# kostastril/Aiyagari-Replication

Hardware: AMD Instinct MI355X
Metric: Bellman evals/sec (Na·Na'·Nz, fp64) (higher is better)
Workload: dtype f64; 1 GPU; aiyagari_vfi_sweep Na=20000 Nz=7 rouwenhorst (BASELINE configs[1]); Na=20000, Nz=7, search=exhaustive over a' (exact bound-tree screen)

## Files before the change

### aiyagari-replication_amd/csrc/bell_dev.hpp

```cpp
#pragma once
#include <hip/hip_runtime.h>

#include "aiy_common.hpp"

namespace aiy {

constexpr double kTau = 1.4210854715202004e-14;
constexpr double kThr = 0.99999999999999644729;
constexpr float kThr32 = 0.999998092651367f;
constexpr float kBig32 = 1.152921504606847e18f;

typedef float f32x2 __attribute__((ext_vector_type(2)));

__device__ __forceinline__ float f32_up(double x) { return nextafterf((float)x, __builtin_inff()); }
__device__ __forceinline__ float f32_dn(double x) { return nextafterf((float)x, -__builtin_inff()); }

template <int NP>
__device__ __forceinline__ f32x2 ipow2(f32x2 c) {
    static_assert(NP >= 1 && NP <= 8, "screen exponent");
    if constexpr (NP == 1) return c;
    f32x2 c2 = c * c;
    if constexpr (NP == 2) return c2;
    if constexpr (NP == 3) return c2 * c;
    f32x2 c4 = c2 * c2;
    if constexpr (NP == 4) return c4;
    if constexpr (NP == 5) return c4 * c;
    if constexpr (NP == 6) return c4 * c2;
    if constexpr (NP == 7) return (c4 * c2) * c;
    return c4 * c4;
}

template <int NP, bool LAB>
__device__ __forceinline__ double bell_val(double c, double ev, double sigma, double dis) {
    double u;
    if constexpr (NP > 0) {
        double p = 1.0 / aiy_ipow(c, NP);
        if constexpr ((NP & (NP - 1)) == 0)
            u = (p - 1) * (-1.0 / NP);
        else
            u = (p - 1) / (1 - sigma);
    } else {
        if (!LAB && sigma == 1.0) u = aiy_log(c);
        else u = (aiy_pow(c, 1.0 - sigma) - 1) / (1 - sigma);
    }
    if constexpr (LAB) return (u - dis) + ev;
    else return u + ev;
}

#define AIY_SCHED_BARRIER() __builtin_amdgcn_sched_barrier(0)
template <int NP, int M, bool CLAMP = true>
__device__ __forceinline__ void screen_t(double (&t)[M], const double (&cx)[M],
                                         const double (&dd)[M]) {
    double c[M], p[M];
#pragma unroll
    for (int m = 0; m < M; ++m) c[m] = CLAMP ? fmax(cx[m], 0.0) : cx[m];
    if constexpr (CLAMP) AIY_SCHED_BARRIER();
#pragma unroll
    for (int m = 0; m < M; ++m) p[m] = c[m];
    constexpr int top = 31 - __builtin_clz((unsigned)NP);
#pragma unroll
    for (int b = top - 1; b >= 0; --b) {
#pragma unroll
        for (int m = 0; m < M; ++m) p[m] = p[m] * p[m];
        AIY_SCHED_BARRIER();
        if ((NP >> b) & 1) {
#pragma unroll
            for (int m = 0; m < M; ++m) p[m] = p[m] * c[m];
            AIY_SCHED_BARRIER();
        }
    }
#pragma unroll
    for (int m = 0; m < M; ++m) t[m] = dd[m] * p[m];
}
__device__ __forceinline__ double clamp0_d(double x) {
#if defined(__HIP_DEVICE_COMPILE__)
    double r;
    asm("v_max_f64 %0, %1, 0" : "=v"(r) : "v"(x));
    return r;
#else
    return fmax(x, 0.0);
#endif
}
template <int RL>
struct StageGroup {
    static constexpr int G = RL <= 2 ? 8 : (RL <= 4 ? 4 : 1);
};

__device__ __forceinline__ bool lexi_take(double val, int q, double& best, int& idx) {
    if (val != val) return false;
    if (idx < 0 || val > best || (val == best && q < idx)) {
        best = val;
        idx = q;
        return true;
    }
    return false;
}

__device__ __forceinline__ void lexi_take_sel(double val, int q, double& best, int& idx) {
    const bool take = (val == val) & ((idx < 0) | (val > best) | ((val == best) & (q < idx)));
    best = take ? val : best;
    idx = take ? q : idx;
}

__device__ __forceinline__ double screen_B(double best, int idx, double dis, int np) {
    if (idx < 0) return -__builtin_inf();
    double nd = (double)np;
    return nd * (best + dis) - kTau * nd * (fabs(best) + fabs(dis));
}

__device__ __forceinline__ double wave_fmin_d(double x) {
    x = fmin(x, dpp_d<0xB1>(x));
    x = fmin(x, dpp_d<0x4E>(x));
    x = fmin(x, dpp_d<0x141>(x));
    x = fmin(x, dpp_d<0x140>(x));
    x = fmin(x, dpp_d<0x142, 0xa>(x));
    x = fmin(x, dpp_d<0x143, 0xc>(x));
    return readlane_d(x, 63);
}
__device__ __forceinline__ double wave_fmax_d(double x) {
    x = fmax(x, dpp_d<0xB1>(x));
    x = fmax(x, dpp_d<0x4E>(x));
    x = fmax(x, dpp_d<0x141>(x));
    x = fmax(x, dpp_d<0x140>(x));
    x = fmax(x, dpp_d<0x142, 0xa>(x));
    x = fmax(x, dpp_d<0x143, 0xc>(x));
    return readlane_d(x, 63);
}

constexpr int kTreeGroup = 8;

__device__ __forceinline__ double group_fmin_d(double x) {
    x = fmin(x, dpp_d<0xB1>(x));
    x = fmin(x, dpp_d<0x4E>(x));
    return fmin(x, dpp_d<0x141>(x));
}
__device__ __forceinline__ double group_fmax_d(double x) {
    x = fmax(x, dpp_d<0xB1>(x));
    x = fmax(x, dpp_d<0x4E>(x));
    return fmax(x, dpp_d<0x141>(x));
}
__device__ __forceinline__ double wave_rest_fmin_d(double x) {
    x = fmin(x, dpp_d<0x140>(x));
    x = fmin(x, dpp_d<0x142, 0xa>(x));
    x = fmin(x, dpp_d<0x143, 0xc>(x));
    return readlane_d(x, 63);
}
__device__ __forceinline__ double wave_rest_fmax_d(double x) {
    x = fmax(x, dpp_d<0x140>(x));
    x = fmax(x, dpp_d<0x142, 0xa>(x));
    x = fmax(x, dpp_d<0x143, 0xc>(x));
    return readlane_d(x, 63);
}

template <int NP>
__device__ __forceinline__ bool screen_wave(double dmax, double a0, double bmin, double cmax) {
    const double cx[1] = {cmax - a0}, dd[1] = {dmax - bmin};
    double t[1];
    screen_t<NP, 1>(t, cx, dd);
    return t[0] >= kThr;
}

template <bool LAB>
__device__ __forceinline__ double cash(double x, double y, double Ll) {
    if constexpr (LAB) return x + y * Ll;
    else return x + y;
}

__device__ __forceinline__ double table_ev(int N, int Na, const double* __restrict__ P,
                                           const double* __restrict__ V, double beta, int i,
                                           int k) {
    double acc = 0.0;
    for (int m0 = 0; m0 < N; m0 += 8) {
        double pm[8], vv[8];
#pragma unroll
        for (int u = 0; u < 8; ++u) {
            const int m = min(m0 + u, N - 1);
            pm[u] = P[i * N + m];
            vv[u] = V[(size_t)m * Na + k];
        }
#pragma unroll
        for (int u = 0; u < 8; ++u) {
            const double term = (beta * pm[u]) * vv[u];
            acc = acc + (m0 + u < N ? term : 0.0);
        }
    }
    return acc;
}
__device__ __forceinline__ double table_D(double ev, int np) {
    double ne = (double)np * ev;
    return (ne + 1.0) + kTau * (fabs(ne) + 1.0);
}

}
```

### aiyagari-replication_amd/csrc/bellman_kernels.hip

```cpp
#include <hip/hip_ext.h>

#include <algorithm>
#include <type_traits>

#include "aiy_common.hpp"
#include "bell_dev.hpp"
#include "bellman.hpp"

namespace aiy {

__device__ __forceinline__ BellArgs bell_cand(const BellArgs& A, int c) {
    BellArgs B = A;
    const size_t o = (size_t)c * A.N * A.Na;
    B.r = A.rv[c];
    B.w = A.wv[c];
    B.v_old += o;
    B.EV += o;
    if (B.Dt) B.Dt += o;
    if (B.Dm8) B.Dm8 += (size_t)c * A.N * A.nb8;
    if (B.Dm512) B.Dm512 += (size_t)c * A.N * A.nb512;
    B.kf += o * A.Nl;
    B.best0 += o;
    B.idx0 += o;
    if (B.hint) B.hint += o;
// ... 537 lines not shown
        const int gb = (k_lo >> 6) + g + lane;
        const bool okb = g + lane < nbk;
        const double dmv = okb ? Dmrow[gb] : -__builtin_inf();
        const double a0v = okb ? a[gb << 6] : 0.0;
        double smv = dmv;
        smv = fmax(smv, __shfl_xor(smv, 1));
        smv = fmax(smv, __shfl_xor(smv, 2));
        smv = fmax(smv, __shfl_xor(smv, 4));
        const int ng = min(64, nbk - g);
        for (int sb = 0; sb < ng; sb += 8) {
            ++nsup;
            if (!bound_pass(readlane_d(smv, sb), readlane_d(a0v, sb))) continue;
            const int se = min(sb + 8, ng);
            for (int b = sb; b < se; ++b) {
                if (se - sb > 1) {
                    ++nblk;
                    if (!bound_pass(readlane_d(dmv, b), readlane_d(a0v, b))) continue;
                }
                const int b0 = k_lo + ((g + b) << 6);
                fine(b0, min(b0 + 64, k_hi));
            }
        }
    }
    if (A.hitcount) {
        const unsigned ns = 64 * R * (l1 - l0);
        nsup *= ns;
        nblk *= ns;
    }

    const size_t slab = ((size_t)lbk * nchunk + chunk) * N + i;
#pragma unroll
    for (int r = 0; r < R; ++r) {
        int j = jbase + r * 64 + lane;
        if (j < Na && imp[r] >= 0) {
            A.partial[slab * Na + j] = imp[r];
            A.touched[(size_t)i * Na + j] = 1;
        }
    }
    if (A.hitcount) {
        unsigned long long* hc = A.hitcount + 4 * (item % kDiffSlots);
        if (nhits) atomicAdd(hc, (unsigned long long)nhits);
        if (lane == 0) {
            atomicAdd(hc + 1, (unsigned long long)nsup);
            atomicAdd(hc + 2, (unsigned long long)nblk);
            if (nfine) atomicAdd(hc + 3, (unsigned long long)nfine * 64 * R * (l1 - l0));
        }
    }
}

template <int NP, bool LAB, int R, int LB, int W, bool INS, int PK, bool HY = false, int WM = 8>
__device__ __forceinline__ void bell_tree_item(const BellArgs& A0, int ntile, int block_id,
                                               int nblocks, double2 (*s_cand)[512],
                                               unsigned long long* s_pass) {
    static_assert(PK == 1 || W == 1, "packed workgroups hold one-wave tiles");
    const int lane = threadIdx.x & 63;
    const int lw = readfirst(threadIdx.x >> 6);
    const int wave = PK > 1 ? 0 : lw;
    asm volatile("" ::"s"(A0.a), "s"(A0.Dt), "s"(A0.EV), "s"(A0.kf), "s"(A0.hint), "s"(A0.v_old),
                 "s"(A0.Dm512), "s"(A0.s), "s"(A0.r), "s"(A0.w), "s"(A0.N), "s"(A0.Na),
                 "s"(A0.variant), "s"(A0.C), "s"(A0.nb512), "s"(A0.sigma), "s"(A0.trace),
                 "s"(A0.best0), "s"(A0.idx0), "s"(A0.tw), "s"(ntile), "s"(nblocks), "s"(A0.mom),
                 "s"(A0.idx), "s"(A0.pk), "s"(A0.pc), "s"(A0.v_new), "s"(A0.diff));
    const long long t_boot = (INS && A0.trace) ? (long long)wall_clock64() : 0;
    const long long c_boot = (INS && A0.trace) ? (long long)__builtin_amdgcn_s_memtime() : 0;
    int item = A0.perm ? A0.perm[block_id]
                       : ((A0.variant & kVarXcdOrder) ? xcd_remap(block_id, nblocks) : block_id);
    if (PK > 1 && item < 0) return;
    BellArgs A = A0;
    if (A0.C > 1) {
        const int c = item / (A0.N * ntile);
        if (A0.stop[c]) return;
        A = bell_cand(A0, c);
        item -= c * A0.N * ntile;
    }
    const int tile = item % ntile;
    const int i = item / ntile;
    const int N = A.N, Na = A.Na, Nl = LAB ? A.Nl : 1;
    const size_t nall = (size_t)N * Na;
    const double* __restrict__ a = A.a;
    const double* __restrict__ Drow = A.Dt + (size_t)i * Na;
    const double* __restrict__ ev = A.EV + (size_t)i * Na;
    const double y = A.w * A.s[i];
    const int TW = (R == 1 && A0.tw > 0) ? A0.tw : 64 * R;
    const int jbase = tile * TW;
    constexpr bool LEAN = (W >= 2 && !HY) || LAB;

    int* __restrict__ mom = (A.variant & kVarNoMomentum) ? nullptr : A.mom;
    constexpr bool PRE = WM == 1;
    int h_pre[R], m_pre[R], kf_pre[R];
    double aj_pre[R];
    if constexpr (PRE) {
#pragma unroll
        for (int r = 0; r < R; ++r) {
            const int j = jbase + r * 64 + lane;
            const int jc = (j < Na && r * 64 + lane < TW) ? j : 0;
            const size_t t = (size_t)i * Na + jc;
            h_pre[r] = A.hint ? A.hint[t] : -1;
            m_pre[r] = (A.hint && mom) ? mom[t] : 0;
            kf_pre[r] = A.kf[t];
            aj_pre[r] = a[jc];
        }
    }
    double dm0_pre, a0_pre;
    {
        const bool oks = lane < A.nb512;
        dm0_pre = oks ? A.Dm512[(size_t)i * A.nb512 + lane] : -__builtin_inf();
        a0_pre = oks ? a[lane << 9] : 0.0;
    }
    double vo_pre[R];
#pragma unroll
    for (int r = 0; r < R; ++r) {
        const int j = jbase + r * 64 + lane;
        vo_pre[r] = (j < Na && r * 64 + lane < TW && wave == 0) ? A.v_old[(size_t)i * Na + j] : 0.0;
    }

    double x[R], best[R];
    int idx[R], hk0[R], mlast[R];
    bool okr[R], feas[R];
    unsigned nsu = 0;
#pragma unroll
    for (int r = 0; r < R; ++r) {
        const int j = jbase + r * 64 + lane;
        okr[r] = j < Na && r * 64 + lane < TW;
        const size_t t = (size_t)i * Na + (okr[r] ? j : 0);
        if constexpr (PRE) x[r] = okr[r] ? (1 + A.r) * aj_pre[r] : 0.0;
        else x[r] = okr[r] ? (1 + A.r) * a[j] : 0.0;
        best[r] = __builtin_nan("");
        idx[r] = -1;
        hk0[r] = -1;
        mlast[r] = 0;
        feas[r] = false;
        if (!okr[r]) continue;
        if constexpr (PRE) feas[r] = kf_pre[r] > 0;
        for (int l = PRE ? 1 : 0; l < Nl; ++l) feas[r] = feas[r] || A.kf[l * nall + t] > 0;
        if (A.hint) {
            int h;
            if constexpr (PRE) h = h_pre[r];
            else h = A.hint[t];
            int mraw = 0;
            if constexpr (PRE) mraw = h >= 0 ? m_pre[r] : 0;
            else mraw = (mom && h >= 0) ? mom[t] : 0;
            const int ms0 = (int)(short)(mraw & 0xffff), ms1 = (int)(short)(mraw >> 16);
            mlast[r] = ms0;
            const int mv = max(-Na, min(Na, (A.variant & kVarDriftExtrap) ? 2 * ms0 - ms1 : ms0));
            if (h >= 0) {
                const int hl = h % Nl;
                const int kf = (PRE && hl == 0) ? kf_pre[r] : A.kf[hl * nall + t];
                if (kf > 0) {
                    const int hk = min(h / Nl, kf - 1);
                    const double coh = cash<LAB>(x[r], y, LAB ? A.L[hl] : 1.0);
                    const double dis = LAB ? A.dis[hl] : 0.0;
                    auto take = [&](int k) __attribute__((always_inline)) {
                        if (INS) ++nsu;
                        return lexi_take(bell_val<NP, LAB>(coh - a[k], ev[k], A.sigma, dis),
                                         hl + Nl * k, best[r], idx[r]);
                    };
                    const int wn =
                        WM == 1 ? 1 : 1 << ((A.variant & kVarHintWinMask) >> kVarHintWinShift);
                    hk0[r] = hk;
                    const int hm = min(max(hk + mv, 0), kf - 1);
                    constexpr int mw = 1;
                    const bool usem = hm > hk + wn + mw || hm < hk - wn - mw;
                    const int wnh = (usem && (A.variant & kVarHintAlone)) ? 0 : wn;
                    const bool skiph = usem && (A.variant & kVarNoHintEval);
                    double wa[2 * WM + 1], we[2 * WM + 1], ma[3], me[3];
#pragma unroll
                    for (int d = -WM; d <= WM; ++d) {
                        if (d < -wnh || d > wnh || skiph) continue;
                        const int kc = min(max(hk + d, 0), kf - 1);
                        wa[d + WM] = a[kc];
                        we[d + WM] = ev[kc];
                    }
                    if (usem) {
#pragma unroll
                        for (int d = -1; d <= 1; ++d) {
                            const int kc = min(max(hm + d, 0), kf - 1);
                            ma[d + 1] = a[kc];
                            me[d + 1] = ev[kc];
                        }
                    }
#pragma unroll
                    for (int d = -WM; d <= WM; ++d) {
                        if (d < -wnh || d > wnh || skiph) continue;
                        const int kc = min(max(hk + d, 0), kf - 1);
                        if (INS) ++nsu;
                        lexi_take(bell_val<NP, LAB>(coh - wa[d + WM], we[d + WM], A.sigma, dis),
                                  hl + Nl * kc, best[r], idx[r]);
                    }
                    if (usem) {
#pragma unroll
                        for (int d = -1; d <= 1; ++d) {
                            const int kc = min(max(hm + d, 0), kf - 1);
                            if (INS) ++nsu;
                            lexi_take(bell_val<NP, LAB>(coh - ma[d + 1], me[d + 1], A.sigma, dis),
                                      hl + Nl * kc, best[r], idx[r]);
                        }
                    }
                    const int kb = idx[r] >= 0 ? idx[r] / Nl : hk;
                    int dir = kb >= hk + wnh ? 1 : (kb <= hk - wnh ? -1 : 0);
                    if (usem && kb >= hm - mw && kb <= hm + mw)
                        dir = kb == hm + mw ? 1 : (kb == hm - mw ? -1 : 0);
                    if (dir != 0 && !(A.variant & kVarNoClimb)) {
                        int k = kb, step = 2;
                        for (;;) {
                            const int kn = min(max(k + dir * step, 0), kf - 1);
                            if (kn == k || !take(kn)) break;
                            k = kn;
                            step <<= 1;
                        }
                        for (int s2 = step >> 1; s2 >= 1; s2 >>= 1) {
                            const int c0 = idx[r] / Nl;
                            if (c0 + s2 < kf) take(c0 + s2);
                            if (c0 - s2 >= 0) take(c0 - s2);
                        }
                    }
                }
            }
        } else {
            best[r] = A.best0[t];
            idx[r] = A.idx0[t] == -2 ? -1 : A.idx0[t];
        }
    }
    int q_su[R];
    double kp_su[R];
#pragma unroll
    for (int r = 0; r < R; ++r) {
        q_su[r] = idx[r];
        kp_su[r] = a[idx[r] >= 0 ? idx[r] / Nl : 0];
    }
    unsigned nhits = nsu, nsup = 0, nwv = 0, nblk = 0, ngt = 0, nfine = 0, lane_pairs = 0;
    unsigned npath[2] = {0, 0};
    const long long t_start = (INS && A.trace) ? (long long)wall_clock64() : 0;
    long long cyc[4] = {0, 0, 0, 0}, c_mark = (INS && A.trace) ? (long long)__builtin_amdgcn_s_memtime() : 0;
    const long long c_mark0 = c_mark;
    auto stamp = [&](int ph) __attribute__((always_inline)) {
        if (INS && A.trace) {
            const long long now = (long long)__builtin_amdgcn_s_memtime();
            cyc[ph] += now - c_mark;
            c_mark = now;
        }
    };
    stamp(0);

    auto exchange = [&]() __attribute__((always_inline)) {
        if constexpr (W > 1) {
#pragma unroll
            for (int r = 0; r < R; ++r)
                s_cand[lw][r * 64 + lane] = make_double2(best[r], (double)idx[r]);
            __syncthreads();
            for (int v = 0; v < W; ++v)
#pragma unroll
                for (int r = 0; r < R; ++r) {
                    const double2 e = s_cand[v][r * 64 + lane];
                    if (v != wave && (int)e.y >= 0) lexi_take(e.x, (int)e.y, best[r], idx[r]);
                }
            __syncthreads();
        }
    };

    for (int l0 = 0; l0 < Nl; l0 += LB) {
        double coh[R][LB], B[R][LB], dis[LB];
        int kg = 0;
        int kfl = 0x7fffffff;
#pragma unroll
        for (int q = 0; q < LB; ++q) dis[q] = (LAB && l0 + q < Nl) ? A.dis[l0 + q] : 0.0;
#pragma unroll
        for (int r = 0; r < R; ++r) {
            const size_t t = (size_t)i * Na + (okr[r] ? jbase + r * 64 + lane : 0);
#pragma unroll
            for (int q = 0; q < LB; ++q) {
                const bool okq = okr[r] && l0 + q < Nl;
                coh[r][q] = okq ? cash<LAB>(x[r], y, LAB ? A.L[l0 + q] : 1.0) : 0.0;
                if (okq) {
                    const int kfv = A.kf[(l0 + q) * nall + t];
                    kg = max(kg, kfv);
                    kfl = min(kfl, kfv);
                }
            }
        }
        constexpr bool FAST = !LAB && R == 1;
        int kfmin = 0;
        if constexpr (FAST)
            if (!(A.variant & kVarPlainScreens)) kfmin = min(wave_min_i32(kfl), Na);
        if (A.r > -1.0) {
            const int jl = min(Na - 1, jbase + TW - 1);
            kg = readlane_i(kg, (jl - jbase) & 63);
        } else {
            for (int off = 32; off > 0; off >>= 1) kg = max(kg, __shfl_xor(kg, off));
            kg = readfirst(kg);
        }
        if (kg == 0) continue;
        if (l0 > 0) exchange();
        auto set_B = [&]() __attribute__((always_inline)) {
#pragma unroll
            for (int r = 0; r < R; ++r)
#pragma unroll
                for (int q = 0; q < LB; ++q)
                    B[r][q] = (okr[r] && l0 + q < Nl) ? screen_B(best[r], idx[r], dis[q], NP)
                                                      : __builtin_nan("");
        };
        set_B();
        constexpr bool GRP = !LAB;
        constexpr int GL = kTreeGroup;
        double gB = __builtin_nan(""), gC = -__builtin_inf();
        auto set_G = [&]() __attribute__((always_inline)) {
            double bl = __builtin_nan(""), cl = -__builtin_inf();
#pragma unroll
            for (int r = 0; r < R; ++r)
#pragma unroll
                for (int q = 0; q < LB; ++q) {
                    bl = fmin(bl, B[r][q]);
                    cl = fmax(cl, (okr[r] && l0 + q < Nl) ? coh[r][q] : -__builtin_inf());
                }
            gB = group_fmin_d(bl);
            gC = group_fmax_d(cl);
        };
        if constexpr (GRP) set_G();

        constexpr int RL = R * LB, G = LEAN ? (RL <= 2 ? 4 : 1) : StageGroup<RL>::G;
        auto mask8 = [&](double dv, double av, int l0, int stride, int cnt, bool sub = false)
                         __attribute__((always_inline)) {
            double dmax[8], a0[8];
#pragma unroll
            for (int u = 0; u < 8; ++u) {
                const int ln = min(l0 + stride * u, 63);
                dmax[u] = readlane_d(dv, ln);
                a0[u] = readlane_d(av, ln);
            }
            bool pu[8];
#pragma unroll
            for (int g0 = 0; g0 < 8; g0 += G) {
                double cx[G * RL], dd[G * RL], t[G * RL];
#pragma unroll
                for (int gu = 0; gu < G; ++gu)
#pragma unroll
                    for (int r = 0; r < R; ++r)
#pragma unroll
                        for (int q = 0; q < LB; ++q) {
                            const int m = (gu * R + r) * LB + q;
                            cx[m] = coh[r][q] - a0[g0 + gu];
                            dd[m] = dmax[g0 + gu] - B[r][q];
                        }
                AIY_SCHED_BARRIER();
                screen_t<NP, G * RL>(t, cx, dd);
#pragma unroll
                for (int gu = 0; gu < G; ++gu) {
                    bool pass = false;
#pragma unroll
                    for (int m = gu * RL; m < (gu + 1) * RL; ++m) pass = pass || t[m] >= kThr;
                    pu[g0 + gu] = pass;
                }
            }
            unsigned m = 0;
#pragma unroll
            for (int u = 0; u < 8; ++u) m |= (__any(pu[u]) ? 1u : 0u) << u;
            if (INS && A.trace && sub)
#pragma unroll
                for (int u = 0; u < 8; ++u) lane_pairs += (u < cnt && pu[u]) ? 1u : 0u;
            return m & ((1u << cnt) - 1u);
        };
        auto load_tk = [&](int bit, double2 (&tk)[8]) __attribute__((always_inline)) {
#pragma unroll
            for (int kk = 0; kk < 8; ++kk) tk[kk] = s_cand[lw][(bit << 3) + kk];
        };
        auto fine = [&](int sbase, int k0, int k1, const double2 (&tk)[8])
                        __attribute__((always_inline)) {
            if (INS && (A.hitcount || A.trace)) nfine += k1 - k0;
            const bool ncl = FAST && k0 + 8 <= kfmin;
            if (INS && A.hitcount) npath[0] += ncl ? 0u : 1u, npath[1] += ncl ? 1u : 0u;
            bool pk[8];
#pragma unroll
            for (int g0 = 0; g0 < 8; g0 += G) {
                double cx[G * RL], dd[G * RL], t[G * RL];
#pragma unroll
                for (int gk = 0; gk < G; ++gk)
#pragma unroll
                    for (int r = 0; r < R; ++r)
#pragma unroll
                        for (int q = 0; q < LB; ++q) {
                            const int m = (gk * R + r) * LB + q;
                            cx[m] = coh[r][q] - tk[g0 + gk].x;
                            dd[m] = tk[g0 + gk].y - B[r][q];
                        }
                AIY_SCHED_BARRIER();
                if constexpr (FAST) {
                    if (!ncl) {
#pragma unroll
                        for (int m = 0; m < G * RL; ++m) cx[m] = clamp0_d(cx[m]);
                        AIY_SCHED_BARRIER();
                    }
                    screen_t<NP, G * RL, false>(t, cx, dd);
                } else {
                    screen_t<NP, G * RL>(t, cx, dd);
                }
#pragma unroll
                for (int gk = 0; gk < G; ++gk) {
                    bool pass = false;
#pragma unroll
                    for (int r = 0; r < R; ++r)
#pragma unroll
                        for (int q = 0; q < LB; ++q) {
                            const int lin = (l0 + q) + Nl * (k0 + g0 + gk);
                            pass = pass || (t[(gk * R + r) * LB + q] >= kThr && lin != idx[r]);
                        }
                    pk[g0 + gk] = pass;
                }
            }
            {
                bool pall = false;
#pragma unroll
                for (int kk = 0; kk < 8; ++kk) pall = pall || pk[kk];
                if (!__any(pall)) return;
            }
            unsigned vote = 0;
#pragma unroll
            for (int kk = 0; kk < 8; ++kk) vote |= (__any(pk[kk]) ? 1u : 0u) << kk;
            vote &= (1u << (k1 - k0)) - 1u;
            if (!vote) return;
            stamp(2);
            while (vote) {
                const int kk = __builtin_ctz(vote);
                vote &= vote - 1;
                const int k = k0 + kk;
                const double2 tkk = s_cand[lw][k - sbase];
#pragma unroll
                for (int r = 0; r < R; ++r)
#pragma unroll
                    for (int q = 0; q < LB; ++q) {
                        const double c = coh[r][q] - tkk.x;
                        const int lin = (l0 + q) + Nl * k;
                        if (lin != idx[r] && c > 0 &&
                            (tkk.y - B[r][q]) * aiy_ipow(c, NP) >= kThr) {
                            ++nhits;
                            const double val =
                                bell_val<NP, LAB>(c, ev[k], A.sigma, dis[q]);
                            if (lexi_take(val, lin, best[r], idx[r])) {
#pragma unroll
                                for (int q2 = 0; q2 < LB; ++q2)
                                    if (B[r][q2] == B[r][q2])
                                        B[r][q2] = screen_B(best[r], idx[r], dis[q2], NP);
                            }
                        }
                    }
            }
            stamp(3);
        };
        auto load8 = [&](int sb, double& dm8, double& a8) __attribute__((always_inline)) {
            const int sub = (sb << 6) + lane;
            const bool oku = sub < A.nb8;
            dm8 = oku ? A.Dm8[(size_t)i * A.nb8 + sub] : -__builtin_inf();
            a8 = oku ? a[sub << 3] : 0.0;
        };
        auto stage = [&](int sbase, unsigned long long pass, double2 (&st)[8])
                         __attribute__((always_inline)) {
            if constexpr (LEAN) {
                unsigned bm = 0;
#pragma unroll
                for (int b = 0; b < 8; ++b) bm |= ((pass >> (8 * b)) & 0xffull) ? 1u << b : 0u;
                while (bm) {
                    const int b0 = __builtin_ctz(bm);
                    bm &= bm - 1;
                    const int b1 = bm ? __builtin_ctz(bm) : -1;
                    if (bm) bm &= bm - 1;
                    const int k0 = min(sbase + (b0 << 6) + lane, Na - 1);
                    const double2 v0 = make_double2(a[k0], Drow[k0]);
                    double2 v1 = make_double2(0.0, 0.0);
                    if (b1 >= 0) {
                        const int k1 = min(sbase + (b1 << 6) + lane, Na - 1);
                        v1 = make_double2(a[k1], Drow[k1]);
                    }
                    s_cand[lw][(b0 << 6) + lane] = v0;
                    if (b1 >= 0) s_cand[lw][(b1 << 6) + lane] = v1;
                }
            } else {
#pragma unroll
                for (int b = 0; b < 8; ++b)
                    if ((pass >> (8 * b)) & 0xffull) {
                        const int k = min(sbase + (b << 6) + lane, Na - 1);
                        st[b] = make_double2(a[k], Drow[k]);
                    }
            }
        };
        auto prep = [&](int sb, int bsel, int bstep, double dm8, double a8, double2 (&st)[8],
                        bool subsplit = false)
                        __attribute__((always_inline)) -> unsigned long long {
            stamp(0);
            const int sbase = sb << 9;
            if constexpr (GRP) {
                constexpr int NG = 64 / GL, CH = LEAN ? 4 : 8;
                static_assert(NG % CH == 0, "whole chunks of groups");
                unsigned long long any = 0;
#pragma unroll
                for (int g0 = 0; g0 < NG; g0 += CH) {
                    double cx[CH], dd[CH], t[CH];
#pragma unroll
                    for (int u = 0; u < CH; ++u) {
                        cx[u] = readlane_d(gC, (g0 + u) * GL) - a8;
                        dd[u] = dm8 - readlane_d(gB, (g0 + u) * GL);
                    }
                    AIY_SCHED_BARRIER();
                    screen_t<NP, CH>(t, cx, dd);
#pragma unroll
                    for (int u = 0; u < CH; ++u) any |= __ballot(t[u] >= kThr);
                }
                if (INS && (A.hitcount || A.trace)) ngt += NG;
                const int nfe = min(64, (kg - sbase + 7) >> 3);
                unsigned long long pass = any & (nfe >= 64 ? ~0ull : (1ull << nfe) - 1ull);
                if (bstep > 1) {
                    const unsigned long long one = subsplit ? 0x01ull : 0xffull;
                    unsigned long long pat = one << (subsplit ? bsel : 8 * bsel);
                    for (int sh = subsplit ? bstep : 8 * bstep; sh < 64; sh <<= 1) pat |= pat << sh;
                    pass &= pat;
                }
                if (INS && (A.hitcount || A.trace)) nblk += __builtin_popcountll(pass);
                unsigned long long keep = 0;
                for (unsigned long long m = pass; m; m &= m - 1) {
                    const int u = __builtin_ctzll(m);
                    const double dv = readlane_d(dm8, u), av = readlane_d(a8, u);
                    double cx[RL], dd[RL], t[RL];
#pragma unroll
                    for (int r = 0; r < R; ++r)
#pragma unroll
                        for (int q = 0; q < LB; ++q) {
                            cx[r * LB + q] = coh[r][q] - av;
                            dd[r * LB + q] = dv - B[r][q];
                        }
                    screen_t<NP, RL>(t, cx, dd);
                    bool p = false;
#pragma unroll
                    for (int m2 = 0; m2 < RL; ++m2) p = p || t[m2] >= kThr;
                    if (__any(p)) keep |= 1ull << u;
                }
                pass = keep;
                if (INS && A.trace && lane == 0) lane_pairs += __builtin_popcountll(pass);
                stage(sbase, pass, st);
                stamp(1);
                return pass;
            }
            double dm64 = dm8;
            dm64 = fmax(dm64, dpp_d<0xB1>(dm64));
            dm64 = fmax(dm64, dpp_d<0x4E>(dm64));
            dm64 = fmax(dm64, dpp_d<0x104>(dm64));
            const int nblock = min(8, (kg - sbase + 63) >> 6);
            unsigned own = 0;
            for (int b = subsplit ? 0 : bsel; b < nblock; b += subsplit ? 1 : bstep) own |= 1u << b;
            if (INS && (A.hitcount || A.trace)) nblk += __builtin_popcount(own);
            const unsigned bpass = mask8(dm64, a8, 0, 8, nblock) & own;
            unsigned long long pass = 0;
            const bool deal = subsplit && bstep > 1;
            int ord = 0;
            for (unsigned bm = bpass; bm; bm &= bm - 1, ++ord) {
                if (deal && ord % bstep != bsel) continue;
                const int b = __builtin_ctz(bm);
                const int nsub = min(8, (kg - (sbase + (b << 6)) + 7) >> 3);
                if (INS && (A.hitcount || A.trace)) nblk += nsub;
                pass |= (unsigned long long)mask8(dm8, a8, 8 * b, 1, nsub, true) << (8 * b);
            }
            if constexpr (W > 1) {
                if (deal) {
                    s_pass[bsel] = pass;
                    __syncthreads();
                    unsigned long long all = 0;
                    for (int v = 0; v < bstep; ++v) all |= s_pass[v];
                    __syncthreads();
                    const unsigned long long pat = bstep == 2 ? 0x5555555555555555ull
                                                 : (bstep == 4 ? 0x1111111111111111ull
                                                               : 0x0101010101010101ull);
                    pass = all & (pat << bsel);
                }
            }
            stage(sbase, pass, st);
            stamp(1);
            return pass;
        };
        auto finish = [&](int sb, unsigned long long pass, const double2 (&st)[8])
                          __attribute__((always_inline)) {
            const int sbase = sb << 9;
            if constexpr (!LEAN)
#pragma unroll
                for (int b = 0; b < 8; ++b)
                    if ((pass >> (8 * b)) & 0xffull) s_cand[lw][(b << 6) + lane] = st[b];
            __builtin_amdgcn_wave_barrier();
            __builtin_amdgcn_fence(__ATOMIC_RELEASE, "wavefront");
            stamp(1);
            double2 tkA[8], tkB[8];
            unsigned long long pm = pass;
            if constexpr (LEAN) {
                for (; pm; pm &= pm - 1) {
                    const int b0 = __builtin_ctzll(pm);
                    load_tk(b0, tkA);
                    fine(sbase, sbase + (b0 << 3), min(sbase + (b0 << 3) + 8, kg), tkA);
                }
            }
            if (pm) load_tk(__builtin_ctzll(pm), tkA);
            while (pm) {
                const int b0 = __builtin_ctzll(pm);
                pm &= pm - 1;
                if (pm) load_tk(__builtin_ctzll(pm), tkB);
                fine(sbase, sbase + (b0 << 3), min(sbase + (b0 << 3) + 8, kg), tkA);
                if (!pm) break;
                const int b1 = __builtin_ctzll(pm);
                pm &= pm - 1;
                if (pm) load_tk(__builtin_ctzll(pm), tkA);
                fine(sbase, sbase + (b1 << 3), min(sbase + (b1 << 3) + 8, kg), tkB);
            }
            stamp(2);
            __builtin_amdgcn_wave_barrier();
        };

        const int nsb = (kg + 511) >> 9;
        int sfirst = -1;
        {
            int hk = -1;
#pragma unroll
            for (int r = 0; r < R; ++r)
                if (idx[r] >= 0) hk = idx[r] / Nl;
            const unsigned long long m = __ballot(hk >= 0);
            if (m) sfirst = min(readlane_i(hk, __builtin_ctzll(m)) >> 9, nsb - 1);
        }
        double2 st_cur[8], st_prev[8];
        if (sfirst >= 0) {
            if (INS) ++nsup;
            double d8, a8;
            load8(sfirst, d8, a8);
            const unsigned long long p = prep(sfirst, wave, W, d8, a8, st_cur,
                                              (A.variant & kVarDealBlocks) != 0);
            if (p) finish(sfirst, p, st_cur);
            exchange();
            set_B();
        }
        double dm0, a0;
        auto load512 = [&](int g) __attribute__((always_inline)) {
            const int sbl = g + lane;
            const bool oks = sbl < nsb;
            dm0 = oks ? A.Dm512[(size_t)i * A.nb512 + sbl] : -__builtin_inf();
            a0 = oks ? a[sbl << 9] : 0.0;
        };
        if (l0 == 0) {
            dm0 = dm0_pre;
            a0 = a0_pre;
        } else {
            load512(0);
        }
        double bmin, cmax;
        {
            if constexpr (GRP) {
                if (sfirst >= 0) set_G();
                bmin = wave_rest_fmin_d(gB);
                cmax = wave_rest_fmax_d(gC);
            } else {
                double bl = __builtin_nan(""), cl = -__builtin_inf();
#pragma unroll
                for (int r = 0; r < R; ++r)
#pragma unroll
                    for (int q = 0; q < LB; ++q) {
                        bl = fmin(bl, B[r][q]);
                        cl = fmax(cl, (okr[r] && l0 + q < Nl) ? coh[r][q] : -__builtin_inf());
                    }
                bmin = wave_fmin_d(bl);
                cmax = wave_fmax_d(cl);
            }
        }
        int g = 0;
        unsigned long long sm = 0;
        auto test512 = [&]() __attribute__((always_inline)) {
            if (INS) ++nwv;
            unsigned long long m =
                __ballot(lane < nsb - g && screen_wave<NP>(dm0, a0, bmin, cmax));
            static_assert(64 % W == 0, "superblock g + u belongs to wave u % W");
            if constexpr (W > 1) m &= (~0ull / ((1ull << W) - 1ull)) << wave;
            if (sfirst >= g && sfirst < g + 64) m &= ~(1ull << (sfirst - g));
            return m;
        };
        if (nsb > 0) sm = test512();
        auto next_sb = [&]() __attribute__((always_inline)) -> int {
            for (;;) {
                if (sm) {
                    const int u = __builtin_ctzll(sm);
                    sm &= sm - 1;
                    if (INS) ++nsup;
                    return g + u;
                }
                g += 64;
                if (g >= nsb) return -1;
                load512(g);
                sm = test512();
            }
        };
        int cur = nsb > 0 ? next_sb() : -1;
        double pd = 0.0, pa = 0.0;
        if (cur >= 0) load8(cur, pd, pa);
        unsigned long long pass_prev = 0;
        int sb_prev = -1;
        while (cur >= 0) {
            const double d8 = pd, a8 = pa;
            const int nxt = next_sb();
            if (nxt >= 0) load8(nxt, pd, pa);
            const unsigned long long pc = prep(cur, 0, 1, d8, a8, st_cur);
            if constexpr (LEAN) {
                if (pc) finish(cur, pc, st_cur);
                cur = nxt;
                continue;
            }
            if (pass_prev) finish(sb_prev, pass_prev, st_prev);
#pragma unroll
            for (int b = 0; b < 8; ++b) st_prev[b] = st_cur[b];
            pass_prev = pc;
            sb_prev = cur;
            cur = nxt;
        }
        if (pass_prev) finish(sb_prev, pass_prev, st_prev);
    }

    exchange();
    const long long c_end = (INS && A.trace) ? (long long)__builtin_amdgcn_s_memtime() : 0;

    bool okd = false;
    double dmax = 0.0;
#pragma unroll
    for (int r = 0; r < R; ++r) {
        if (!okr[r] || wave != 0) continue;
        const size_t t = (size_t)i * Na + jbase + r * 64 + lane;
        double b = best[r];
        int q = idx[r];
        const double vo = vo_pre[r];
        if (!feas[r] && LAB) {
            b = A.keep_incoming ? A.v_new[t] : vo;
        } else {
            if (q < 0) {
                q = 0;
                b = __builtin_nan("");
            }
            const int l = q % Nl, k = q / Nl;
            double kp = kp_su[r];
            if (__ballot(q != q_su[r]) != 0ull) kp = a[k];
            A.idx[t] = q;
            if (A.pk) A.pk[t] = kp;
            if (A.pc) A.pc[t] = cash<LAB>(x[r], y, LAB ? A.L[l] : 1.0) - kp;
            if (LAB && A.pl) A.pl[t] = A.L[l];
        }
        A.v_new[t] = b;
        if (mom && A.hint) {
            const int sh = (hk0[r] >= 0 && idx[r] >= 0) ? idx[r] / Nl - hk0[r] : 0;
            const int shc = max(-32767, min(32767, sh));
            mom[t] = (int)(((unsigned)shc & 0xffffu) | ((unsigned)mlast[r] << 16));
        }
        const double d = fabs(b - vo);
        if (d == d) {
            dmax = okd ? fmax(dmax, d) : d;
            okd = true;
        }
    }
    if constexpr (W == 1) wave_max_to_slots(okd, dmax, A.diff);
    else block_max_to_slots(okd, dmax, A.diff);
    if (INS && A.trace) {
        __shared__ unsigned s_cnt[W][4];
        __shared__ unsigned s_pairs;
        static_assert(LAB || 8 % (R * LB) == 0, "group tests in whole block-test units");
        const unsigned nblk_all = nblk + ngt / (R * LB);
        unsigned pairs = lane_pairs, sums[4] = {nsup, nblk_all, nfine, nhits};
        if constexpr (W == 1) {
            for (int o = 32; o > 0; o >>= 1) pairs += __shfl_xor(pairs, o);
        } else {
            if (threadIdx.x == 0) s_pairs = 0;
            __syncthreads();
            atomicAdd(&s_pairs, lane_pairs);
            if (lane == 0) {
                s_cnt[wave][0] = nsup; s_cnt[wave][1] = nblk_all; s_cnt[wave][2] = nfine; s_cnt[wave][3] = nhits;
            }
            __syncthreads();
            pairs = s_pairs;
            for (int c = 0; c < 4; ++c) {
                unsigned sum = 0;
                for (int v = 0; v < W; ++v) sum += s_cnt[v][c];
                sums[c] = sum;
            }
        }
        if (W == 1 ? lane == 0 : threadIdx.x == 0) {
            long long* tr = A.trace + 16 * (size_t)item;
            tr[0] = t_start;
            tr[1] = (long long)wall_clock64();
            tr[2] = (long long)(unsigned)__builtin_amdgcn_s_getreg((20 << 0) | (0 << 6) | (3 << 11)) |
                    ((long long)(unsigned)__builtin_amdgcn_s_getreg((4 << 0) | (0 << 6) | (31 << 11))
                     << 32);
            for (int c = 0; c < 4; ++c) tr[3 + c] = sums[c];
            tr[7] = block_id;
            for (int c = 0; c < 4; ++c) tr[8 + c] = cyc[c];
            tr[12] = t_boot;
            tr[13] = c_mark0 - c_boot;
            tr[14] = (long long)__builtin_amdgcn_s_memtime() - c_end;
            tr[15] = pairs;
        }
    }
    if (INS && A.hitcount) {
        unsigned long long* hc = A.hitcount + 4 * (blockIdx.x % kDiffSlots);
        if (nhits) atomicAdd(hc, (unsigned long long)nhits);
        if (lane == 0) {
            const unsigned long long ns = 64ull * R * LB;
            atomicAdd(hc + 1, nwv * 64ull);
            atomicAdd(hc + 2, nblk * ns + ngt * 64ull);
            if (nfine) atomicAdd(hc + 3, nfine * ns);
#pragma unroll
            for (int q = 0; q < 2; ++q)
                if (npath[q]) atomicAdd(hc + kPathBase + q, (unsigned long long)npath[q]);
        }
    }
}

template <int NP, bool LAB, int R, int LB, int W, bool INS, int PK, int WM>
__global__ __launch_bounds__(64 * W * PK, 3) void bell_tree_kernel(BellArgs A0, int ntile) {
    __shared__ double2 s_cand[W * PK][512];
    __shared__ unsigned long long s_pass[W];
    const int lw = PK > 1 ? readfirst(threadIdx.x >> 6) : 0;
    bell_tree_item<NP, LAB, R, LB, W, INS, PK, false, WM>(A0, ntile, (int)blockIdx.x * PK + lw,
                                                          (int)gridDim.x * PK, s_cand, s_pass);
}

template <int NP, bool INS>
__global__ __launch_bounds__(128, 3) void bell_tree_hybrid_kernel(BellArgs A0, int ntile) {
    __shared__ double2 s_cand[2][512];
    __shared__ unsigned long long s_pass[2];
    const int b = (int)blockIdx.x;
    if (A0.perm[2 * b + 1] == -2) {
        bell_tree_item<NP, false, 1, 1, 2, INS, 1, true>(A0, ntile, 2 * b, 2 * (int)gridDim.x,
                                                        s_cand, s_pass);
    } else {
        const int lw = readfirst(threadIdx.x >> 6);
        bell_tree_item<NP, false, 1, 1, 1, INS, 2, true>(A0, ntile, 2 * b + lw,
                                                        2 * (int)gridDim.x, s_cand, s_pass);
    }
}

template <int NP, bool LAB, int LB>
__global__ void bell_merge_kernel(BellArgs A, int use_partial, int nlb, int nchunk) {
    int t = blockIdx.x * blockDim.x + threadIdx.x;
    bool ok = false;
    double d = 0.0;
    const int N = A.N, Na = A.Na, Nl = A.Nl;
    if (t < N * Na) {
        int i = t / Na, j = t - i * Na;
        const double* __restrict__ a = A.a;
        double x = (1 + A.r) * a[j];
        double y = A.w * A.s[i];
        double best = A.best0[t];
        int idx = A.idx0[t];
        if (use_partial && A.touched[t]) {
            A.touched[t] = 0;
            const double* __restrict__ ev = A.EV + (size_t)i * Na;
            for (int lbk = 0; lbk < nlb; ++lbk) {
                int kfm = 0;
                for (int l = lbk * LB; l < min(lbk * LB + LB, Nl); ++l)
                    kfm = max(kfm, A.kf[(size_t)l * N * Na + t]);
                int nch = (kfm + A.CK - 1) / A.CK;
                for (int c = 0; c < nch; ++c) {
                    int* pq = A.partial + (((size_t)lbk * nchunk + c) * N + i) * Na + j;
                    int q = *pq;
                    if (q >= 0) {
                        *pq = -1;
                        int l = q % Nl, k = q / Nl;
                        double coh = cash<LAB>(x, y, LAB ? A.L[l] : 1.0);
                        lexi_take(bell_val<NP, LAB>(coh - a[k], ev[k], A.sigma,
                                                    LAB ? A.dis[l] : 0.0),
                                  q, best, idx);
                    }
                }
            }
        }
        double vo = A.v_old[t];
        if (idx == -2 && LAB) {
            best = A.keep_incoming ? A.v_new[t] : vo;
        } else {
            if (idx < 0) {
                idx = 0;
                best = __builtin_nan("");
            }
            int l = idx % Nl, k = idx / Nl;
            double kp = a[k];
            double coh = cash<LAB>(x, y, LAB ? A.L[l] : 1.0);
            A.idx[t] = idx;
            if (A.pk) A.pk[t] = kp;
            if (A.pc) A.pc[t] = coh - kp;
            if (LAB && A.pl) A.pl[t] = A.L[l];
        }
        A.v_new[t] = best;
        d = fabs(best - vo);
        ok = (d == d);
    }
    block_max_to_slots(ok, d, A.diff);
}

template <int NP, bool LAB>
__global__ __launch_bounds__(256) void bell_plain_kernel(BellArgs A) {
    constexpr int W = 4, U = 8;
    __shared__ double s_best[W][64];
    __shared__ int s_idx[W][64];
    const int lane = threadIdx.x & 63;
    const int wave = __builtin_amdgcn_readfirstlane(threadIdx.x >> 6);
    const int Na = A.Na, Nl = A.Nl;
    const int i = blockIdx.y;
    const int j = blockIdx.x * 64 + lane;
    const bool okj = j < Na;
    const size_t t = (size_t)i * Na + (okj ? j : 0);
    const double* __restrict__ a = A.a;
    const double* __restrict__ ev = A.EV + (size_t)i * Na;
    const double x = okj ? (1 + A.r) * a[j] : 0.0, y = A.w * A.s[i];
    double best = __builtin_nan("");
    int idx = -1;
    bool anyfeas = false;
    for (int l = 0; l < Nl; ++l) {
        const double coh = cash<LAB>(x, y, LAB ? A.L[l] : 1.0);
        const double dis = LAB ? A.dis[l] : 0.0;
        const int kf = okj ? A.kf[(size_t)l * A.N * Na + t] : 0;
        anyfeas = anyfeas || kf > 0;
        int km = kf;
        for (int off = 32; off > 0; off >>= 1) km = max(km, __shfl_xor(km, off));
        const int kmax = __builtin_amdgcn_readfirstlane(km);
        const int kc = (kmax + W * U - 1) / (W * U) * U;
        const int k_lo = wave * kc, k_hi = min(kmax, k_lo + kc);
        for (int k = k_lo; k < k_hi; k += U) {
            double v[U];
#pragma unroll
            for (int u = 0; u < U; ++u) {
                const int kk = min(k + u, Na - 1);
                const double val = bell_val<NP, LAB>(coh - a[kk], ev[kk], A.sigma, dis);
                v[u] = (k + u < kf) ? val : __builtin_nan("");
            }
            AIY_SCHED_BARRIER();
#pragma unroll
            for (int u = 0; u < U; ++u) lexi_take_sel(v[u], l + Nl * (k + u), best, idx);
        }
    }
    s_best[wave][lane] = best;
    s_idx[wave][lane] = idx;
    __syncthreads();
    bool okd = false;
    double dd = 0.0;
    if (wave == 0 && okj) {
#pragma unroll
        for (int w = 1; w < W; ++w) lexi_take(s_best[w][lane], s_idx[w][lane], best, idx);
        const double vo = A.v_old[t];
        if (!anyfeas && LAB) {
            best = A.keep_incoming ? A.v_new[t] : vo;
        } else {
            if (idx < 0) {
                idx = 0;
                best = __builtin_nan("");
            }
            const int l = idx % Nl, k = idx / Nl;
            const double kp = a[k];
            A.idx[t] = idx;
            if (A.pk) A.pk[t] = kp;
            if (A.pc) A.pc[t] = cash<LAB>(x, y, LAB ? A.L[l] : 1.0) - kp;
            if (LAB && A.pl) A.pl[t] = A.L[l];
        }
        A.v_new[t] = best;
        dd = fabs(best - vo);
        okd = dd == dd;
    }
    block_max_to_slots(okd, dd, A.diff);
}

static inline int cdiv(long long a, long long b) { return (int)((a + b - 1) / b); }

thread_local DispatchEvents g_dispatch_ev;

int launch_bell_ev_mfma(const BellArgs& A, hipStream_t st) {
    const dim3 grid(cdiv(A.Na, 64), cdiv(A.N, 16), std::max(A.C, 1));
    bell_ev_mfma_kernel<<<grid, 256, 0, st>>>(A.N, A.Na, A.P, A.v_old, A.beta, A.EV,
                                              A.C > 1 ? A.stop : nullptr);
    AIY_HIP(hipGetLastError());
    return AIY_OK;
}

int launch_bell_table(const BellArgs& A, hipStream_t st) {
    static_assert(2 * kDiffSlots <= kTableBlock, "table block clears the diff slots");
    dim3 grid(cdiv(A.Na, kTableBlock), A.N);
    const bool scr = A.np > 0;
    if (A.ev_mfma) AIY_TRY(launch_bell_ev_mfma(A, st));
    bell_table_kernel<<<grid, kTableBlock, 0, st>>>(
        A.N, A.Na, A.P, A.v_old, A.beta, A.np, A.a, A.EV, (scr && !A.tree) ? A.T : nullptr,
        scr ? A.T32 : nullptr, A.CK, scr ? A.Dm : nullptr, scr ? A.Dm8 : nullptr,
        scr ? A.Dm512 : nullptr, A.nb, A.nb8, A.nb512, A.diff, scr ? A.Dt : nullptr, A.fold,
        A.ev_mfma, (A.variant & kVarXcdOrder) != 0);
    AIY_HIP(hipGetLastError());
    return AIY_OK;
}

int launch_bell_kf(const BellArgs& A, hipStream_t st) {
    int n = std::max(A.C, 1) * A.N * A.Na * A.Nl;
    if (A.labor) bell_kf_kernel<true><<<cdiv(n, 256), 256, 0, st>>>(A);
    else bell_kf_kernel<false><<<cdiv(n, 256), 256, 0, st>>>(A);
    AIY_HIP(hipGetLastError());
    return AIY_OK;
}

__global__ void kf_tile_last_kernel(const int* __restrict__ kf, int rows, int Na, int TW,
                                    int ntile, int* __restrict__ out) {
    const int g = blockIdx.x * blockDim.x + threadIdx.x;
    if (g >= rows * ntile) return;
    const int row = g / ntile, t = g - row * ntile;
    out[g] = kf[(size_t)row * Na + min(Na - 1, t * TW + TW - 1)];
}
int launch_kf_tile_last(const int* kf, int rows, int Na, int TW, int ntile, int* out,
                        hipStream_t st) {
    kf_tile_last_kernel<<<cdiv((long long)rows * ntile, 256), 256, 0, st>>>(kf, rows, Na, TW,
                                                                             ntile, out);
    AIY_HIP(hipGetLastError());
    return AIY_OK;
}

#ifndef AIY_BELL_R
#define AIY_BELL_R 2
#endif
template <int NP, bool LAB>
// ... 205 lines not shown
```

Measured before the change: 101800 billion evals/s.

## Track per-lane-group block masks so fine screening skips blocks other groups need

In the exhaustive bound-tree screen, prep now also records which 8-lane groups passed each 8-wide block and ORs that mask across each group with DPP. finish then walks each group's own block list, so lanes in different groups process different blocks in the same iteration instead of the whole wave visiting every block any lane needs. The goal is fewer wasted fine-stage iterations on the R==1, W==1, non-LAB path. The cost is more complex control flow, per-lane tail and active masking, and a changed self-exclusion test based on dk, which add risk of divergence overhead or correctness slips.

```diff
diff --git a/aiyagari-replication_amd/csrc/bell_dev.hpp b/aiyagari-replication_amd/csrc/bell_dev.hpp
--- a/aiyagari-replication_amd/csrc/bell_dev.hpp
+++ b/aiyagari-replication_amd/csrc/bell_dev.hpp
@@ -139,6 +139,15 @@
     x = fmax(x, dpp_d<0x4E>(x));
     return fmax(x, dpp_d<0x141>(x));
 }
+constexpr int kFineGroup = 8;
+
+__device__ __forceinline__ unsigned long long group_or_u64(unsigned long long m) {
+    static_assert(kFineGroup == 8 || kFineGroup == 64, "the ladder is written for eight lanes");
+    m |= dpp_u64<0xB1>(m);
+    m |= dpp_u64<0x4E>(m);
+    return m | dpp_u64<0x141>(m);
+}
+
 __device__ __forceinline__ double wave_rest_fmin_d(double x) {
     x = fmin(x, dpp_d<0x140>(x));
     x = fmin(x, dpp_d<0x142, 0xa>(x));
diff --git a/aiyagari-replication_amd/csrc/bellman_kernels.hip b/aiyagari-replication_amd/csrc/bellman_kernels.hip
--- a/aiyagari-replication_amd/csrc/bellman_kernels.hip
+++ b/aiyagari-replication_amd/csrc/bellman_kernels.hip
@@ -863,6 +863,7 @@
         set_B();
         constexpr bool GRP = !LAB;
         constexpr int GL = kTreeGroup;
+        constexpr bool GF = GRP && W == 1 && R == 1 && !LEAN && !HY && kFineGroup < 64;
         double gB = __builtin_nan(""), gC = -__builtin_inf();
         auto set_G = [&]() __attribute__((always_inline)) {
             double bl = __builtin_nan(""), cl = -__builtin_inf();
@@ -924,10 +925,15 @@
 #pragma unroll
             for (int kk = 0; kk < 8; ++kk) tk[kk] = s_cand[lw][(bit << 3) + kk];
         };
-        auto fine = [&](int sbase, int k0, int k1, const double2 (&tk)[8])
-                        __attribute__((always_inline)) {
-            if (INS && (A.hitcount || A.trace)) nfine += k1 - k0;
-            const bool ncl = FAST && k0 + 8 <= kfmin;
+        auto fine = [&](int sbase, int k0, int k1, const double2 (&tk)[8], bool act = true,
+                        bool ncl_sb = false) __attribute__((always_inline)) {
+            if (INS && (A.hitcount || A.trace)) {
+                if constexpr (GF)
+                    nfine += readlane_i(min(8, kg - k0), __builtin_ctzll(__ballot(act)));
+                else nfine += k1 - k0;
+            }
+            const bool ncl = GF ? ncl_sb : (FAST && k0 + 8 <= kfmin);
+            const int dk = GF ? idx[0] - k0 : 0;
             if (INS && A.hitcount) npath[0] += ncl ? 0u : 1u, npath[1] += ncl ? 1u : 0u;
             bool pk[8];
 #pragma unroll
@@ -961,8 +967,12 @@
                     for (int r = 0; r < R; ++r)
 #pragma unroll
                         for (int q = 0; q < LB; ++q) {
-                            const int lin = (l0 + q) + Nl * (k0 + g0 + gk);
-                            pass = pass || (t[(gk * R + r) * LB + q] >= kThr && lin != idx[r]);
+                            if constexpr (GF) {
+                                pass = pass || (t[(gk * R + r) * LB + q] >= kThr && dk != g0 + gk);
+                            } else {
+                                const int lin = (l0 + q) + Nl * (k0 + g0 + gk);
+                                pass = pass || (t[(gk * R + r) * LB + q] >= kThr && lin != idx[r]);
+                            }
                         }
                     pk[g0 + gk] = pass;
                 }
@@ -971,12 +981,14 @@
                 bool pall = false;
 #pragma unroll
                 for (int kk = 0; kk < 8; ++kk) pall = pall || pk[kk];
-                if (!__any(pall)) return;
+                if (!__any(GF ? pall && act : pall)) return;
             }
             unsigned vote = 0;
-#pragma unroll
-            for (int kk = 0; kk < 8; ++kk) vote |= (__any(pk[kk]) ? 1u : 0u) << kk;
-            vote &= (1u << (k1 - k0)) - 1u;
+            const int nk = GF ? (act ? kg - k0 : 0) : 8;
+#pragma unroll
+            for (int kk = 0; kk < 8; ++kk)
+                vote |= (__any(GF ? pk[kk] && kk < nk : pk[kk]) ? 1u : 0u) << kk;
+            if constexpr (!GF) vote &= (1u << (k1 - k0)) - 1u;
             if (!vote) return;
             stamp(2);
             while (vote) {
@@ -990,7 +1002,7 @@
                     for (int q = 0; q < LB; ++q) {
                         const double c = coh[r][q] - tkk.x;
                         const int lin = (l0 + q) + Nl * k;
-                        if (lin != idx[r] && c > 0 &&
+                        if (lin != idx[r] && c > 0 && (!GF || kk < nk) &&
                             (tkk.y - B[r][q]) * aiy_ipow(c, NP) >= kThr) {
                             ++nhits;
                             const double val =
@@ -1043,7 +1055,7 @@
             }
         };
         auto prep = [&](int sb, int bsel, int bstep, double dm8, double a8, double2 (&st)[8],
-                        bool subsplit = false)
+                        unsigned long long& gmo, bool subsplit = false)
                         __attribute__((always_inline)) -> unsigned long long {
             stamp(0);
             const int sbase = sb << 9;
@@ -1074,7 +1086,7 @@
                     pass &= pat;
                 }
                 if (INS && (A.hitcount || A.trace)) nblk += __builtin_popcountll(pass);
-                unsigned long long keep = 0;
+                unsigned long long keep = 0, own = 0;
                 for (unsigned long long m = pass; m; m &= m - 1) {
                     const int u = __builtin_ctzll(m);
                     const double dv = readlane_d(dm8, u), av = readlane_d(a8, u);
@@ -1091,8 +1103,10 @@
 #pragma unroll
                     for (int m2 = 0; m2 < RL; ++m2) p = p || t[m2] >= kThr;
                     if (__any(p)) keep |= 1ull << u;
+                    if constexpr (GF) own |= p ? 1ull << u : 0ull;
                 }
                 pass = keep;
+                if constexpr (GF) gmo = keep ? group_or_u64(own) : 0ull;
                 if (INS && A.trace && lane == 0) lane_pairs += __builtin_popcountll(pass);
                 stage(sbase, pass, st);
                 stamp(1);
@@ -1134,8 +1148,8 @@
             stamp(1);
             return pass;
         };
-        auto finish = [&](int sb, unsigned long long pass, const double2 (&st)[8])
-                          __attribute__((always_inline)) {
+        auto finish = [&](int sb, unsigned long long pass, const double2 (&st)[8],
+                          unsigned long long gm) __attribute__((always_inline)) {
             const int sbase = sb << 9;
             if constexpr (!LEAN)
 #pragma unroll
@@ -1153,6 +1167,35 @@
                     fine(sbase, sbase + (b0 << 3), min(sbase + (b0 << 3) + 8, kg), tkA);
                 }
             }
+            if constexpr (GF) {
+                pm = 0;
+                const int hb = 63 - __builtin_clzll(pass);
+                const bool ncl = FAST && sbase + (hb << 3) + 8 <= kfmin;
+                auto next = [&](int& k0) __attribute__((always_inline)) {
+                    const unsigned lo = (unsigned)gm, hi = (unsigned)(gm >> 32);
+                    const unsigned tl = lo ? (unsigned)__builtin_ctz(lo) : ~0u;
+                    const unsigned th = hi ? ((unsigned)__builtin_ctz(hi) | 32u) : ~0u;
+                    const int b = (int)min(min(tl, th), (unsigned)hb);
+                    gm &= gm - 1;
+                    k0 = sbase + (b << 3);
+                    return b;
+                };
+                int kA, kB;
+                bool actA = gm != 0, actB;
+                load_tk(next(kA), tkA);
+                for (;;) {
+                    actB = gm != 0;
+                    const bool moreB = __any(actB);
+                    if (moreB) load_tk(next(kB), tkB);
+                    fine(sbase, kA, 0, tkA, actA, ncl);
+                    if (!moreB) break;
+                    actA = gm != 0;
+                    const bool moreA = __any(actA);
+                    if (moreA) load_tk(next(kA), tkA);
+                    fine(sbase, kB, 0, tkB, actB, ncl);
+                    if (!moreA) break;
+                }
+            }
             if (pm) load_tk(__builtin_ctzll(pm), tkA);
             while (pm) {
                 const int b0 = __builtin_ctzll(pm);
@@ -1184,9 +1227,10 @@
             if (INS) ++nsup;
             double d8, a8;
             load8(sfirst, d8, a8);
-            const unsigned long long p = prep(sfirst, wave, W, d8, a8, st_cur,
+            unsigned long long gm1 = 0;
+            const unsigned long long p = prep(sfirst, wave, W, d8, a8, st_cur, gm1,
                                               (A.variant & kVarDealBlocks) != 0);
-            if (p) finish(sfirst, p, st_cur);
+            if (p) finish(sfirst, p, st_cur, gm1);
             exchange();
             set_B();
         }
@@ -1251,26 +1295,27 @@
         int cur = nsb > 0 ? next_sb() : -1;
         double pd = 0.0, pa = 0.0;
         if (cur >= 0) load8(cur, pd, pa);
-        unsigned long long pass_prev = 0;
+        unsigned long long pass_prev = 0, gm_cur = 0, gm_prev = 0;
         int sb_prev = -1;
         while (cur >= 0) {
             const double d8 = pd, a8 = pa;
             const int nxt = next_sb();
             if (nxt >= 0) load8(nxt, pd, pa);
-            const unsigned long long pc = prep(cur, 0, 1, d8, a8, st_cur);
+            const unsigned long long pc = prep(cur, 0, 1, d8, a8, st_cur, gm_cur);
             if constexpr (LEAN) {
-                if (pc) finish(cur, pc, st_cur);
+                if (pc) finish(cur, pc, st_cur, gm_cur);
                 cur = nxt;
                 continue;
             }
-            if (pass_prev) finish(sb_prev, pass_prev, st_prev);
+            if (pass_prev) finish(sb_prev, pass_prev, st_prev, gm_prev);
 #pragma unroll
             for (int b = 0; b < 8; ++b) st_prev[b] = st_cur[b];
             pass_prev = pc;
+            gm_prev = gm_cur;
             sb_prev = cur;
             cur = nxt;
         }
-        if (pass_prev) finish(sb_prev, pass_prev, st_prev);
+        if (pass_prev) finish(sb_prev, pass_prev, st_prev, gm_prev);
     }
 
     exchange();
```

Result: faster. 105600 billion evals/s (median of 6 runs) (+3.8%).
